# yuxng/PoseCNN

Hardware: NVIDIA H100
Metric: frames/sec on 640x480 RGB, 21 classes, batch 32 (VGG16 + Hough + ROI pose head) (higher is better)
Workload: dtype bf16 operands / fp32 accumulate (conv stack, 1x1 heads), fp16 operands / fp32 accumulate (fc6-fc8), fp32 / int32 elsewhere

## Files before the change

include/posecnn_b200.h:

```cpp
#ifndef POSECNN_B200_H_
#define POSECNN_B200_H_

#include <stddef.h>
#include <stdint.h>

#ifdef __cplusplus
extern "C" {
#endif

#define PCNN_OK 0
#define PCNN_E_INVALID (-1)
#define PCNN_E_WORKSPACE (-2)
#define PCNN_E_CUDA (-3)

#define PCNN_MAX_ROI 128
#define PCNN_HOUGH_MAX_ROWS (PCNN_MAX_ROI * 9)

const char* pcnn_last_error(void);
int pcnn_version(void);

int pcnn_hough_vote_workspace_bytes(int B, int H, int W, int C, int skip_pixels, float threshold_vote,
                                    size_t* bytes);
int pcnn_hough_vote_fwd(const int32_t* label, const float* vertex, const float* extents, const float* meta,
                        const float* gt, int B, int H, int W, int C, int num_gt, int num_meta, int is_train,
// ... 21 lines not shown
                           int height, int width, int channels, int pooled_height, int pooled_width,
                           float spatial_scale, float* top, int32_t* argmax, void* stream);
int pcnn_roi_pool_bwd(const float* top_diff, const int32_t* argmax, const float* rois, int batch, int num_rois,
                      int channel_rois, int height, int width, int channels, int pooled_height,
                      int pooled_width, float spatial_scale, int pool_channel, float* bottom_diff,
                      void* stream);

int pcnn_hard_label_fwd(const float* prob, const int32_t* gt, int B, int H, int W, int C, float threshold,
                        float* top, void* stream);
int pcnn_hard_label_bwd(int B, int H, int W, int C, float* grad_prob, float* grad_gt, void* stream);

int pcnn_backproject_fwd(const float* data, const float* label, const float* depth, const float* meta,
                         const float* label_3d, int B, int H, int W, int Cf, int C, int num_meta,
                         int grid_size, int kernel_size, float threshold, float* top_data, float* top_label,
                         float* top_flag, void* stream);
int pcnn_backproject_bwd(const float* top_diff, const float* depth, const float* meta, int B, int H, int W,
                         int Cf, int num_meta, int grid_size, float* bottom_diff, void* stream);

int pcnn_project_fwd(const float* data, const float* depth, const float* meta, int B, int H, int W, int Cf,
                     int num_meta, int grid_size, float* top, void* stream);
int pcnn_project_bwd(const float* top_diff, const float* depth, const float* meta, int B, int H, int W, int Cf,
                     int num_meta, int grid_size, int kernel_size, float threshold, float* bottom_diff,
                     void* stream);

int pcnn_average_distance_workspace_bytes(int N, size_t* bytes);
int pcnn_average_distance_fwd(const float* prediction, const float* target, const float* weight,
                              const float* point, const float* symmetry, int N, int C, int P, float margin,
                              float* loss, float* bottom_diff, void* workspace, size_t workspace_bytes,
                              void* stream);
int pcnn_average_distance_bwd(const float* top_diff, const float* bottom_diff, int N, int channels,
                              float* output, void* stream);

int pcnn_conv_bf16_tc(const void* in_bf16, const void* weights_bf16, const float* bias, void* out_bf16, int B,
                      int H, int W, int Cin, int Cout, int ksize, int relu, int block_n, void* stream);
int pcnn_conv_pool_bf16_tc(const void* in_bf16, const void* weights_bf16, const float* bias, void* out_pooled_bf16,
                           int B, int H, int W, int Cin, int Cout, int ksize, int relu, int block_n, void* stream);
int pcnn_conv3x3_small_cin(const float* in, const float* weights_hwio, const float* bias, void* out_bf16, int B,
                           int H, int W, int Cin, int Cout, int relu, void* stream);
int pcnn_im2col_c3(const void* in, int in_is_u8, const float* mean3_host, void* out_bf16, int B, int H, int W,
                   void* stream);
int pcnn_im2col_depth(const float* depth, const float* mean3_host, void* out_bf16, int B, int H, int W, void* stream);
int pcnn_conv1_fused_tc(const void* in, int in_is_u8, const float* mean3_host, const void* weights_bf16,
                        const float* bias, void* out_bf16, int B, int H, int W, int relu, void* stream);
int pcnn_conv1_depth_fused_tc(const float* depth, const float* mean3_host, const void* weights_bf16, const float* bias,
                              void* out_bf16, int B, int H, int W, int relu, void* stream);
int pcnn_maxpool2x2_bf16(const void* in_bf16, void* out_bf16, int B, int H, int W, int C, void* stream);

int pcnn_conv_wgrad_workspace_bytes(int B, int H, int W, int Cin, int Cout, int ksize, size_t* bytes);
int pcnn_conv_wgrad_bf16_tc(const void* x_bf16, const void* dz_bf16, int B, int H, int W, int Cin, int Cout, int ksize,
                            float scale, const float* w_f32, float decay, float* dW, void* workspace, size_t workspace_bytes,
                            void* stream);
int pcnn_fc_wgrad_f16_tc(const void* x_f16, const void* dy_f16, int rows, int Cin, int Cout, float scale, const float* w_f32,
                         float decay, float* dW, void* workspace, size_t workspace_bytes, void* stream);
int pcnn_bias_ws_bytes(int C, size_t* bytes);
int pcnn_relu_bwd_bf16(const void* g_bf16, const void* y_bf16, size_t npix, int C, int has_relu, void* dz_bf16, float scale,
                       const float* b, float decay, float* db, void* bias_ws, size_t bias_ws_bytes, void* stream);
int pcnn_maxpool_relu_bwd_bf16(const void* g_bf16, const void* y_bf16, int B, int H, int W, int C, void* dz_bf16, float scale,
                               const float* b, float decay, float* db, void* bias_ws, size_t bias_ws_bytes, void* stream);
int pcnn_add_to_bf16(const void* a_bf16, const void* b_bf16, const float* b_f32, size_t n, void* out_bf16, void* stream);

int pcnn_add_up2_bf16(const void* a4_bf16, const void* a5_bf16, int B, int h, int w, int C, void* out_bf16, void* stream);
int pcnn_up2_bwd_bf16(const void* dadd_bf16, const void* y5_bf16, int B, int h, int w, int C, void* d5_bf16, void* stream);
int pcnn_pack_lowres(const void* sc_bf16, int Cs, const void* vt_bf16, int Cv, int B, int h, int w, int C, float* lowres, void* stream);
int pcnn_up8_heads_bwd_ex(const float* prob, const float* score, const int32_t* gt, const float* cls_loss_out, float upstream_cls,
                          float threshold, const float* vertex_pred, const float* lowres, const float* bias_vertex, const float* centers,
                          const float* vertex_loss_out, float upstream_vertex, float w_inside, float sigma, int B, int h, int w, int C,
                          int Cs, int Cv, void* d_sc_bf16, void* d_vt_bf16, float* dbias, void* workspace, size_t workspace_bytes,
                          void* stream);
int pcnn_up8_heads_bwd_coord(const float* prob, const float* score, const int32_t* gt, const float* cls_loss_out, float upstream_cls,
// ... 123 lines not shown
```

posecnn_b200/conv.py:

```python
from __future__ import annotations

import torch

from ._lib import check, lib, ptr, stream


def hwio_to_tc(weights_hwio: torch.Tensor, dtype=torch.bfloat16) -> torch.Tensor:
    kh, kw, ci, co = weights_hwio.shape
    return weights_hwio.permute(3, 0, 1, 2).reshape(co, kh * kw * ci).to(dtype).contiguous()


def hwio_to_tc_dgrad(weights_hwio: torch.Tensor) -> torch.Tensor:
    kh, kw, ci, co = weights_hwio.shape
    flipped = torch.flip(weights_hwio, dims=(0, 1)).permute(0, 1, 3, 2).contiguous()
    return hwio_to_tc(flipped)


def conv_bf16(x: torch.Tensor, w_tc: torch.Tensor, bias: torch.Tensor, ksize: int, relu: bool, block_n: int = 0,
              out: torch.Tensor | None = None) -> torch.Tensor:
    assert x.is_cuda and x.dtype == torch.bfloat16 and x.is_contiguous() and x.dim() == 4
    assert w_tc.dtype == torch.bfloat16 and w_tc.is_contiguous() and bias.dtype == torch.float32
    B, H, W, Cin = x.shape
    Cout = w_tc.shape[0]
    assert w_tc.shape[1] == ksize * ksize * Cin
    if out is None:
        out = torch.empty((B, H, W, Cout), dtype=torch.bfloat16, device=x.device)
    check(lib().pcnn_conv_bf16_tc(ptr(x), ptr(w_tc), ptr(bias), ptr(out), B, H, W, Cin, Cout, int(ksize), int(bool(relu)),
                                  int(block_n), stream()))
    return out


def conv_pool_bf16(x: torch.Tensor, w_tc: torch.Tensor, bias: torch.Tensor, ksize: int, relu: bool, block_n: int = 0) -> torch.Tensor:
    assert x.is_cuda and x.dtype == torch.bfloat16 and x.is_contiguous() and x.dim() == 4
    B, H, W, Cin = x.shape
    Cout = w_tc.shape[0]
    out = torch.empty((B, H // 2, W // 2, Cout), dtype=torch.bfloat16, device=x.device)
    check(lib().pcnn_conv_pool_bf16_tc(ptr(x), ptr(w_tc), ptr(bias), ptr(out), B, H, W, Cin, Cout, int(ksize), int(bool(relu)),
                                       int(block_n), stream()))
    return out


def conv3x3_small_cin(x: torch.Tensor, w_hwio: torch.Tensor, bias: torch.Tensor, relu: bool = True) -> torch.Tensor:
    assert x.is_cuda and x.dtype == torch.float32 and x.is_contiguous()
    B, H, W, Cin = x.shape
    Cout = w_hwio.shape[3]
    out = torch.empty((B, H, W, Cout), dtype=torch.bfloat16, device=x.device)
    check(lib().pcnn_conv3x3_small_cin(ptr(x), ptr(w_hwio.contiguous()), ptr(bias), ptr(out), B, H, W, Cin, Cout,
                                       int(bool(relu)), stream()))
    return out


def maxpool2x2(x: torch.Tensor) -> torch.Tensor:
    assert x.is_cuda and x.dtype == torch.bfloat16 and x.is_contiguous()
    B, H, W, C = x.shape
    out = torch.empty((B, H // 2, W // 2, C), dtype=torch.bfloat16, device=x.device)
    check(lib().pcnn_maxpool2x2_bf16(ptr(x), ptr(out), B, H, W, C, stream()))
    return out


def im2col_c3(x: torch.Tensor, mean=None) -> torch.Tensor:
    import ctypes
    assert x.is_cuda and x.is_contiguous() and x.shape[3] == 3 and x.dtype in (torch.float32, torch.uint8)
# ... 45 lines not shown
```

posecnn_b200/csrc/conv_tc.cu:

```cuda
#include <cuda.h>
#include <cuda_bf16.h>

#include <type_traits>

#include "common.cuh"
#include "tc_common.cuh"

namespace pcnn {
namespace convtc {

constexpr int kTileH = 8, kTileW = 16;
static_assert(kTileH * kTileW == kTileM, "pixel tile = two wgmma M blocks");
constexpr int kABytes = kTileM * kKC * 2;
constexpr int kConsumers = 256;
constexpr int kProducerWarp = kConsumers / 32;
constexpr int kThreadsConv = kConsumers + 128;
constexpr int kConsumerRegs = 232, kProducerRegs = 40;
constexpr int kThreadsRow = kConsumers + 32;
constexpr int kStageBytes = 16 * 1024;

struct ConvParams {
    int B, H, W, Cin, Cout;
    int taps, ksize;
    int tiles_h, tiles_w, n_tiles_n, total_tiles;
    int tile_h, tile_w;
    int relu;
    int pool;
    int kc_outer;
    const float* bias;
};

__device__ __forceinline__ void consumer_sync() { asm volatile("bar.sync 1, 256;" ::: "memory"); }

__device__ __forceinline__ void release(uint64_t* bar, int lane)
{
    __syncwarp();
    if (lane == 0) mbar_arrive(bar);
}

__device__ __forceinline__ void stage_rows(uint8_t* ob, const float* a, const float* bias, int relu, int row, int q)
{
#pragma unroll
    for (int i = 0; i < 2; i++) {
        const int r = row + 8 * i;
#pragma unroll
        for (int jj = 0; jj < 8; jj++) {
            const int c = 8 * jj + 2 * q;
            float v0 = a[4 * jj + 2 * i] + __ldg(bias + c), v1 = a[4 * jj + 2 * i + 1] + __ldg(bias + c + 1);
            if (relu) { v0 = fmaxf(v0, 0.f); v1 = fmaxf(v1, 0.f); }
            *reinterpret_cast<uint32_t*>(ob + r * 128 + ((jj ^ (r & 7)) << 4) + 4 * q) = pack_bf16(v0, v1);
        }
    }
}

__device__ __forceinline__ void pool_staged(uint8_t* ob, int t)
{
    const int p = t >> 3, piece = t & 7;
    const int m = 32 * (p >> 3) + 2 * (p & 7);
    const int rows[4] = {m, m + 1, m + 16, m + 17};
    __nv_bfloat162 v[4];
    uint4 x = *reinterpret_cast<const uint4*>(ob + rows[0] * 128 + ((piece ^ (rows[0] & 7)) << 4));
    *reinterpret_cast<uint4*>(v) = x;
#pragma unroll
    for (int k = 1; k < 4; k++) {
        uint4 y = *reinterpret_cast<const uint4*>(ob + rows[k] * 128 + ((piece ^ (rows[k] & 7)) << 4));
        const __nv_bfloat162* yv = reinterpret_cast<const __nv_bfloat162*>(&y);
#pragma unroll
        for (int q = 0; q < 4; q++) v[q] = __hmax2(v[q], yv[q]);
    }
    consumer_sync();
    *reinterpret_cast<uint4*>(ob + p * 128 + ((piece ^ (p & 7)) << 4)) = *reinterpret_cast<const uint4*>(v);
}

template <int BN, int BM>
struct SmemPlan {
    static constexpr int kABytesT = BM * kKC * 2;
    static constexpr int kBBytes = BN * kKC * 2;
    static constexpr int kStage = kABytesT + kBBytes;
    static constexpr int kStages = BN == 256 || BM == 256 ? 4 : (BN == 128 ? 6 : 8);
    static constexpr int kOutBufs = 2;
    static constexpr int kBarOff = kStages * kStage + kOutBufs * kStageBytes;
    static constexpr int kTotal = kBarOff + 256 + 1024;
};

template <int BN, int BM>
__global__ void __launch_bounds__(kThreadsConv, 1)
k_conv_tc(const __grid_constant__ CUtensorMap map_in, const __grid_constant__ CUtensorMap map_w,
          const __grid_constant__ CUtensorMap map_out, const ConvParams p)
{
    static_assert(BM == 128 || (BM == 256 && BN <= 128), "k_conv_tc: BM = 256 needs BN <= 128 (accumulator registers)");
    using Plan = SmemPlan<BN, BM>;
    constexpr int kMB = BM / kTileM;
    extern __shared__ uint8_t smem_raw[];
    uint8_t* smem = reinterpret_cast<uint8_t*>((reinterpret_cast<uintptr_t>(smem_raw) + 1023) & ~(uintptr_t)1023);
    uint8_t* out_stage = smem + Plan::kStages * Plan::kStage;
    uint64_t* full = reinterpret_cast<uint64_t*>(smem + Plan::kBarOff);
    uint64_t* empty = full + Plan::kStages;

    const int warp = threadIdx.x >> 5, lane = threadIdx.x & 31;
    const int kchunks = p.Cin / kKC;
    const int ksteps = p.taps * kchunks;

    if (warp == kProducerWarp && lane == 0) {
        asm volatile("prefetch.tensormap [%0];" ::"l"(&map_in) : "memory");
        asm volatile("prefetch.tensormap [%0];" ::"l"(&map_w) : "memory");
        asm volatile("prefetch.tensormap [%0];" ::"l"(&map_out) : "memory");
        for (int s = 0; s < Plan::kStages; s++) { mbar_init(&full[s], 1); mbar_init(&empty[s], kConsumers / 32); }
        fence_barrier_init();
    }
    __syncthreads();

    if (warp >= kProducerWarp) {
        setmaxnreg_dec<kProducerRegs>();
        if (warp == kProducerWarp && elect_one()) {
            int stage = 0;
            uint32_t phase = 0;
            for (int tile = blockIdx.x; tile < p.total_tiles; tile += gridDim.x) {
                const int nt = tile % p.n_tiles_n;
                int rest = tile / p.n_tiles_n;
                const int tw = rest % p.tiles_w; rest /= p.tiles_w;
                const int th = rest % p.tiles_h;
                const int img = rest / p.tiles_h;
                const int h0 = th * p.tile_h, w0 = tw * p.tile_w, n0 = nt * BN;
                const int pad = p.ksize / 2;
#pragma unroll 1
                for (int ks = 0; ks < ksteps; ks++) {
                    const bool kc_outer = BM == 256 && p.kc_outer;
                    const int tap = kc_outer ? ks % p.taps : ks / kchunks;
                    const int c0 = (kc_outer ? ks / p.taps : ks % kchunks) * kKC;
                    const int dy = tap / p.ksize - pad, dx = tap % p.ksize - pad;
                    mbar_wait(&empty[stage], phase ^ 1);
                    uint8_t* sa = smem + stage * Plan::kStage;
                    mbar_arrive_expect_tx(&full[stage], Plan::kStage);
                    tma_load_4d(sa, &map_in, &full[stage], c0, w0 + dx, h0 + dy, img);
                    tma_load_2d(sa + Plan::kABytesT, &map_w, &full[stage], tap * p.Cin + c0, n0);
                    if (++stage == Plan::kStages) { stage = 0; phase ^= 1; }
                }
            }
        }
    } else {
        setmaxnreg_inc<kConsumerRegs>();
        const int wg = warp >> 2, wq = warp & 3;
        const int row = wg * 64 + wq * 16 + (lane >> 2);
        float acc[kMB][BN / 2];
        int stage = 0, obuf = 0;
        uint32_t phase = 0;
        for (int tile = blockIdx.x; tile < p.total_tiles; tile += gridDim.x) {
            const int nt = tile % p.n_tiles_n;
            int rest = tile / p.n_tiles_n;
            const int tw = rest % p.tiles_w; rest /= p.tiles_w;
            const int th = rest % p.tiles_h;
            const int img = rest / p.tiles_h;
            const int h0 = th * p.tile_h, w0 = tw * p.tile_w, n0 = nt * BN;
            int prev = -1;
            for (int ks = 0; ks < ksteps; ks++) {
                mbar_wait(&full[stage], phase);
                const uint32_t sa = smem_u32(smem + stage * Plan::kStage);
                const uint64_t db = make_desc(sa + Plan::kABytesT);
#pragma unroll
                for (int h = 0; h < kMB; h++) acc_fence<BN / 2>(acc[h]);
                wgmma_fence();
#pragma unroll
                for (int h = 0; h < kMB; h++) {
                    const uint64_t da = make_desc(sa + (h * 2 + wg) * 64 * 128);
#pragma unroll
                    for (int k = 0; k < kKC / 16; k++)
                        wgmma<BN, 0, 0, 0>(acc[h], da + (uint64_t)(k * 2), db + (uint64_t)(k * 2), (ks | k) != 0);
                }
                wgmma_commit();
#pragma unroll
                for (int h = 0; h < kMB; h++) acc_fence<BN / 2>(acc[h]);
                if (prev >= 0) {
                    wgmma_wait<1>();
                    release(&empty[prev], lane);
                }
                prev = stage;
                if (++stage == Plan::kStages) { stage = 0; phase ^= 1; }
            }
            wgmma_wait<0>();
#pragma unroll
            for (int h = 0; h < kMB; h++) acc_fence<BN / 2>(acc[h]);
            release(&empty[prev], lane);
#pragma unroll
            for (int h = 0; h < kMB; h++) {
                if (h > 0 && h0 + 8 * h >= p.H) break;
#pragma unroll
                for (int g = 0; g < BN / 64; g++) {
                    if (threadIdx.x == 0) tma_store_wait_read<1>();
                    consumer_sync();
                    uint8_t* ob = out_stage + obuf * kStageBytes;
                    stage_rows(ob, acc[h] + g * 32, p.bias + n0 + g * 64, p.relu, row, lane & 3);
                    if (p.pool) {
                        consumer_sync();
                        pool_staged(ob, threadIdx.x);
                    }
                    fence_proxy_async();
                    consumer_sync();
                    if (threadIdx.x == 0) {
                        if (!p.pool) tma_store_4d(&map_out, ob, n0 + g * 64, w0, h0 + 8 * h, img);
                        else tma_store_4d(&map_out, ob, n0 + g * 64, w0 >> 1, (h0 >> 1) + 4 * h, img);
                        tma_store_commit();
                    }
                    obuf ^= 1;
                }
            }
        }
        if (threadIdx.x == 0) tma_store_wait_all();
    }
}

constexpr int kRowPx = 128, kPatchW = 130, kPatchH = 4;
constexpr int kPatchBytes = kPatchW * kPatchH * 128;
constexpr int kRowAStages = 2;

template <int BN, bool RESB>
struct RowPlan {
    static constexpr int kBBytes = BN * 128;
    static constexpr int kBStages = RESB ? 9 : 6;
    static constexpr int kBOff = kRowAStages * kPatchBytes;
    static constexpr int kOutOff = kBOff + kBStages * kBBytes;
    static constexpr int kOutBytes = RESB ? kStageBytes : 2 * kStageBytes;
    static constexpr int kBarOff = kOutOff + kOutBytes;
    static constexpr int kTotal = kBarOff + 256 + 1024;
};

template <int BN, bool RESB>
__global__ void __launch_bounds__(kThreadsRow, 1)
k_conv_row2(const __grid_constant__ CUtensorMap map_in , const __grid_constant__ CUtensorMap map_w,
            const __grid_constant__ CUtensorMap map_out ,
            const ConvParams p)
{
    using Plan = RowPlan<BN, RESB>;
    static_assert(BN == 64, "row mode: 64-channel N tiles");
// ... 511 lines not shown
        const size_t n = r / Ho;
        const __nv_bfloat16* p0 = in + ((n * H + 2 * yo) * W + 2 * xo) * C + g * 8;
        uint4 a = __ldg(reinterpret_cast<const uint4*>(p0));
        uint4 b = __ldg(reinterpret_cast<const uint4*>(p0 + C));
        uint4 c = __ldg(reinterpret_cast<const uint4*>(p0 + (size_t)W * C));
        uint4 d = __ldg(reinterpret_cast<const uint4*>(p0 + (size_t)W * C + C));
        uint4 o;
        const __nv_bfloat162* pa = reinterpret_cast<const __nv_bfloat162*>(&a);
        const __nv_bfloat162* pb = reinterpret_cast<const __nv_bfloat162*>(&b);
        const __nv_bfloat162* pc = reinterpret_cast<const __nv_bfloat162*>(&c);
        const __nv_bfloat162* pd = reinterpret_cast<const __nv_bfloat162*>(&d);
        __nv_bfloat162* po = reinterpret_cast<__nv_bfloat162*>(&o);
#pragma unroll
        for (int k = 0; k < 4; k++) po[k] = __hmax2(__hmax2(pa[k], pb[k]), __hmax2(pc[k], pd[k]));
        *reinterpret_cast<uint4*>(out + ((n * Ho + yo) * Wo + xo) * C + g * 8) = o;
    }
}

static int make_map_nhwc(CUtensorMap* m, const void* ptr, int B, int H, int W, int C, int box_c, int box_w = kTileW, int box_h = kTileH)
{
    EncodeTiledFn enc = get_encode();
    if (!enc) { set_error("cuTensorMapEncodeTiled unavailable (driver too old?)"); return PCNN_E_CUDA; }
    cuuint64_t dims[4] = {(cuuint64_t)C, (cuuint64_t)W, (cuuint64_t)H, (cuuint64_t)B};
    cuuint64_t strides[3] = {(cuuint64_t)C * 2, (cuuint64_t)W * C * 2, (cuuint64_t)H * W * C * 2};
    cuuint32_t box[4] = {(cuuint32_t)box_c, (cuuint32_t)box_w, (cuuint32_t)box_h, 1};
    cuuint32_t es[4] = {1, 1, 1, 1};
    CUresult r = enc(m, CU_TENSOR_MAP_DATA_TYPE_BFLOAT16, 4, const_cast<void*>(ptr), dims, strides, box, es,
                     CU_TENSOR_MAP_INTERLEAVE_NONE, CU_TENSOR_MAP_SWIZZLE_128B, CU_TENSOR_MAP_L2_PROMOTION_L2_256B,
                     CU_TENSOR_MAP_FLOAT_OOB_FILL_NONE);
    if (r != CUDA_SUCCESS) { set_error("cuTensorMapEncodeTiled(NHWC %dx%dx%dx%d) failed: %d", B, H, W, C, (int)r); return PCNN_E_CUDA; }
    return PCNN_OK;
}

template <int BN, int BM = kTileM>
static int launch_conv(const CUtensorMap& mi, const CUtensorMap& mw, const CUtensorMap& mo, const ConvParams& p, int num_sms,
                       cudaStream_t st)
{
    using Plan = SmemPlan<BN, BM>;
    PCNN_SMEM_OPTIN((k_conv_tc<BN, BM>), Plan::kTotal, "conv_tc");
    int grid = p.total_tiles < num_sms ? p.total_tiles : num_sms;
    k_conv_tc<BN, BM><<<grid, kThreadsConv, Plan::kTotal, st>>>(mi, mw, mo, p);
    return check_launch("conv_tc");
}

template <int BN, bool RESB>
static int launch_conv_row2(const CUtensorMap& mi, const CUtensorMap& mw, const CUtensorMap& mo, const ConvParams& p, int num_sms,
                            cudaStream_t st)
{
    using Plan = RowPlan<BN, RESB>;
    PCNN_SMEM_OPTIN((k_conv_row2<BN, RESB>), Plan::kTotal, "conv_row2");
    int grid = p.total_tiles < num_sms ? p.total_tiles : num_sms;
    if (RESB) grid = grid / p.n_tiles_n * p.n_tiles_n;
    k_conv_row2<BN, RESB><<<grid, kThreadsRow, Plan::kTotal, st>>>(mi, mw, mo, p);
    return check_launch("conv_row2");
}

}
}

using namespace pcnn;
using namespace pcnn::convtc;

static int conv_bf16_tc_impl(const void* in, const void* weights, const float* bias, void* out, int B, int H, int W, int Cin,
                            int Cout, int ksize, int relu, int block_n, int pool, void* stream);

extern "C" int pcnn_conv_bf16_tc(const void* in, const void* weights, const float* bias, void* out, int B, int H, int W,
                                 int Cin, int Cout, int ksize, int relu, int block_n, void* stream)
{
    return conv_bf16_tc_impl(in, weights, bias, out, B, H, W, Cin, Cout, ksize, relu, block_n, 0, stream);
}

extern "C" int pcnn_conv_pool_bf16_tc(const void* in, const void* weights, const float* bias, void* out_pooled, int B, int H,
                                      int W, int Cin, int Cout, int ksize, int relu, int block_n, void* stream)
{
    PCNN_REQUIRE(H % 2 == 0 && W % 2 == 0, "conv_pool: needs even H, W (got %d x %d)", H, W);
    return conv_bf16_tc_impl(in, weights, bias, out_pooled, B, H, W, Cin, Cout, ksize, relu, block_n, 1, stream);
}

static int conv_bf16_tc_impl(const void* in, const void* weights, const float* bias, void* out, int B, int H, int W, int Cin,
                            int Cout, int ksize, int relu, int block_n, int pool, void* stream)
{
    PCNN_REQUIRE(in && weights && bias && out, "conv: NULL tensor pointer");
    PCNN_REQUIRE(ksize == 1 || ksize == 3, "conv: ksize must be 1 or 3 (got %d)", ksize);
    PCNN_REQUIRE(Cin % 64 == 0 && Cin >= 64, "conv: Cin must be a multiple of 64 (got %d)", Cin);
    PCNN_REQUIRE(Cout % 64 == 0 && Cout >= 64, "conv: Cout must be a multiple of 64 (got %d)", Cout);
    PCNN_REQUIRE(B >= 1 && H >= 1 && W >= 1, "conv: bad shape");
    int bn = block_n;
    if (bn == 0) bn = Cout % 256 == 0 && ksize * ksize * Cin >= 2304 ? 256 : (Cout % 128 == 0 ? 128 : 64);
    PCNN_REQUIRE((bn == 64 || bn == 128 || bn == 256) && Cout % bn == 0, "conv: block_n %d does not divide Cout %d", bn, Cout);
    int dev = 0, sms = kNumSMs;
    cudaGetDevice(&dev);
    cudaDeviceGetAttribute(&sms, cudaDevAttrMultiProcessorCount, dev);
    cudaStream_t st = (cudaStream_t)stream;
    CUtensorMap mi, mw, mo;
    int rc;
    const bool tile256 = block_n == 0 && ksize == 3 && Cin <= 128 && Cout == 128;
    if (block_n == 0 && ksize == 3 && Cin <= 128 && Cout == 64 && H % 2 == 0 && W >= kRowPx) {
        const bool resb = Cin == 64;
        bn = 64;
        rc = make_map_nhwc(&mi, in, B, H, W, Cin, kKC, kPatchW, kPatchH);
        if (rc) return rc;
        rc = make_map_weights(&mw, weights, 9 * Cin, Cout, bn);
        if (rc) return rc;
        rc = pool ? make_map_nhwc(&mo, out, B, H / 2, W / 2, Cout, 64, kRowPx / 2, 1) : make_map_nhwc(&mo, out, B, H, W, Cout, 64, kRowPx, 1);
        if (rc) return rc;
        ConvParams p;
        p.B = B; p.H = H; p.W = W; p.Cin = Cin; p.Cout = Cout; p.ksize = 3; p.taps = 9;
        p.tile_h = 2; p.tile_w = kRowPx;
        p.tiles_h = H / 2;
        p.tiles_w = (W + kRowPx - 1) / kRowPx;
        p.n_tiles_n = Cout / bn;
        p.total_tiles = B * p.tiles_h * p.tiles_w * p.n_tiles_n;
        p.relu = relu; p.pool = pool; p.bias = bias; p.kc_outer = 0;
        if (resb && p.total_tiles >= p.n_tiles_n) return launch_conv_row2<64, true>(mi, mw, mo, p, sms, st);
        return launch_conv_row2<64, false>(mi, mw, mo, p, sms, st);
    }
    int tile_h = kTileH, tile_w = kTileW;
    if (tile256) tile_h = 2 * kTileH;
    else if (!pool && ((H + 15) / 16) * ((W + 7) / 8) < ((H + 7) / 8) * ((W + 15) / 16)) { tile_h = 16; tile_w = 8; }
    rc = make_map_nhwc(&mi, in, B, H, W, Cin, kKC, tile_w, tile_h);
    if (rc) return rc;
    rc = make_map_weights(&mw, weights, ksize * ksize * Cin, Cout, bn);
    if (rc) return rc;
    rc = pool ? make_map_nhwc(&mo, out, B, H / 2, W / 2, Cout, 64, kTileW / 2, kTileH / 2)
              : make_map_nhwc(&mo, out, B, H, W, Cout, 64, tile_w, tile256 ? kTileH : tile_h);
    if (rc) return rc;
    ConvParams p;
    p.B = B; p.H = H; p.W = W; p.Cin = Cin; p.Cout = Cout;
    p.ksize = ksize; p.taps = ksize * ksize;
    p.tile_h = tile_h; p.tile_w = tile_w;
    p.tiles_h = (H + tile_h - 1) / tile_h;
    p.tiles_w = (W + tile_w - 1) / tile_w;
    p.n_tiles_n = Cout / bn;
    p.total_tiles = B * p.tiles_h * p.tiles_w * p.n_tiles_n;
    p.relu = relu;
    p.pool = pool;
    p.bias = bias;
    p.kc_outer = tile256 && H % 2 == 0 && W >= kRowPx;
    if (tile256) return launch_conv<128, 256>(mi, mw, mo, p, sms, st);
    if (bn == 256) return launch_conv<256>(mi, mw, mo, p, sms, st);
    if (bn == 128) return launch_conv<128>(mi, mw, mo, p, sms, st);
    return launch_conv<64>(mi, mw, mo, p, sms, st);
}

extern "C" int pcnn_conv3x3_small_cin(const float* in, const float* weights_hwio, const float* bias, void* out, int B, int H,
                                      int W, int Cin, int Cout, int relu, void* stream)
{
    PCNN_REQUIRE(in && weights_hwio && bias && out, "conv_small: NULL tensor pointer");
    PCNN_REQUIRE(Cin >= 1 && Cin <= 8 && Cout % 16 == 0 && Cout <= 128, "conv_small: needs Cin <= 8, Cout %% 16 == 0, Cout <= 128");
    size_t smem = sizeof(float) * (size_t)(9 * Cin + 1) * Cout;
    size_t total = (size_t)B * H * W * (Cout / 16);
    int blocks = (int)((total + 255) / 256 < (size_t)kNumSMs * 8 ? (total + 255) / 256 : (size_t)kNumSMs * 8);
    k_conv_small_cin<16><<<blocks, 256, smem, (cudaStream_t)stream>>>(in, weights_hwio, bias, (__nv_bfloat16*)out, B, H, W, Cin,
                                                                      Cout, relu);
    return check_launch("conv_small_cin");
}

extern "C" int pcnn_maxpool2x2_bf16(const void* in, void* out, int B, int H, int W, int C, void* stream)
{
    PCNN_REQUIRE(in && out, "maxpool: NULL tensor pointer");
    PCNN_REQUIRE(H % 2 == 0 && W % 2 == 0 && C % 8 == 0, "maxpool: needs even H, W and C %% 8 == 0 (got %d,%d,%d)", H, W, C);
    size_t total = (size_t)B * (H / 2) * (W / 2) * (C / 8);
    int blocks = (int)((total + 255) / 256 < (size_t)kNumSMs * 16 ? (total + 255) / 256 : (size_t)kNumSMs * 16);
    k_maxpool2x2_bf16<<<blocks, 256, 0, (cudaStream_t)stream>>>((const __nv_bfloat16*)in, (__nv_bfloat16*)out, B, H, W, C);
    return check_launch("maxpool2x2");
}

extern "C" int pcnn_im2col_c3(const void* in, int in_is_u8, const float* mean3_host, void* out_bf16, int B, int H, int W,
                              void* stream)
{
    PCNN_REQUIRE(in && out_bf16, "im2col: NULL tensor pointer");
    float m0 = 0.f, m1 = 0.f, m2 = 0.f;
    if (mean3_host) { m0 = mean3_host[0]; m1 = mean3_host[1]; m2 = mean3_host[2]; }
    PCNN_REQUIRE(H <= 65535 && B <= 65535, "im2col: image too tall for the launch grid");
    dim3 grid((W + 127) / 128, H, B);
// ... 21 lines not shown
                            const float* bias, void* out_bf16, int B, int H, int W, int relu, void* stream);

extern "C" int pcnn_conv1_fused_tc(const void* in, int in_is_u8, const float* mean3_host, const void* weights_bf16,
                                   const float* bias, void* out_bf16, int B, int H, int W, int relu, void* stream)
{
    return conv1_fused_impl(in, in_is_u8 ? 1 : 0, mean3_host, weights_bf16, bias, out_bf16, B, H, W, relu, stream);
}

extern "C" int pcnn_conv1_depth_fused_tc(const float* depth, const float* mean3_host, const void* weights_bf16,
                                         const float* bias, void* out_bf16, int B, int H, int W, int relu, void* stream)
{
    return conv1_fused_impl(depth, 2, mean3_host, weights_bf16, bias, out_bf16, B, H, W, relu, stream);
}

static int conv1_fused_impl(const void* in, int in_kind, const float* mean3_host, const void* weights_bf16,
                                   const float* bias, void* out_bf16, int B, int H, int W, int relu, void* stream)
{
    PCNN_REQUIRE(in && weights_bf16 && bias && out_bf16, "conv1: NULL tensor pointer");
    PCNN_REQUIRE(B >= 1 && H >= 1 && W >= 1, "conv1: bad shape");
    float m0 = 0.f, m1 = 0.f, m2 = 0.f;
    if (mean3_host) { m0 = mean3_host[0]; m1 = mean3_host[1]; m2 = mean3_host[2]; }
    CUtensorMap mw, mo;
    int rc = make_map_weights(&mw, weights_bf16, 64, 64, 64);
    if (rc) return rc;
    rc = make_map_nhwc(&mo, out_bf16, B, H, W, 64, 64);
    if (rc) return rc;
    ConvParams p;
    p.B = B; p.H = H; p.W = W; p.Cin = 3; p.Cout = 64; p.ksize = 3; p.taps = 9;
    p.tile_h = kTileH; p.tile_w = kTileW;
    p.tiles_h = (H + kTileH - 1) / kTileH;
    p.tiles_w = (W + kTileW - 1) / kTileW;
    p.n_tiles_n = 1;
    p.total_tiles = B * p.tiles_h * p.tiles_w;
    p.relu = relu; p.pool = 0; p.bias = bias; p.kc_outer = 0;
    int dev = 0, sms = kNumSMs;
    cudaGetDevice(&dev);
    cudaDeviceGetAttribute(&sms, cudaDevAttrMultiProcessorCount, dev);
    int grid = p.total_tiles < sms ? p.total_tiles : sms;
    cudaStream_t st = (cudaStream_t)stream;
    PCNN_SMEM_OPTIN(k_conv1_tc<unsigned char>, kC1Smem, "conv1_tc<u8>");
    PCNN_SMEM_OPTIN(k_conv1_tc<float>, kC1Smem, "conv1_tc<f32>");
    PCNN_SMEM_OPTIN(k_conv1_tc<DepthIn>, kC1Smem, "conv1_tc<depth>");
    if (in_kind == 1) k_conv1_tc<unsigned char><<<grid, kC1Threads, kC1Smem, st>>>((const unsigned char*)in, mw, mo, p, m0, m1, m2);
    else if (in_kind == 2) k_conv1_tc<DepthIn><<<grid, kC1Threads, kC1Smem, st>>>((const DepthIn*)in, mw, mo, p, m0, m1, m2);
    else k_conv1_tc<float><<<grid, kC1Threads, kC1Smem, st>>>((const float*)in, mw, mo, p, m0, m1, m2);
    return check_launch("conv1_fused_tc");
}
```

posecnn_b200/networks/trunk.py:

```python
from __future__ import annotations

import torch

from .. import conv

PIXEL_MEANS = (102.9801, 115.9465, 122.7717)

VGG_CFG = [("conv1_1", 3, 64), ("conv1_2", 64, 64), "pool1", ("conv2_1", 64, 128), ("conv2_2", 128, 128), "pool2",
           ("conv3_1", 128, 256), ("conv3_2", 256, 256), ("conv3_3", 256, 256), "pool3", ("conv4_1", 256, 512),
           ("conv4_2", 512, 512), ("conv4_3", 512, 512), "pool4", ("conv5_1", 512, 512), ("conv5_2", 512, 512),
           ("conv5_3", 512, 512)]


def trunk_shapes(sfx=""):
    shapes = {}
    for item in VGG_CFG:
        if isinstance(item, tuple):
            name, ci, co = item
            shapes[f"{name}{sfx}/weights"] = (3, 3, ci, co)
            shapes[f"{name}{sfx}/biases"] = (co,)
    return shapes


def conv_weights_to_tc(w: torch.Tensor) -> torch.Tensor:
    return conv.conv1_1_weights_to_tc(w) if w.shape[2] == 3 else conv.hwio_to_tc(w)


def run_trunk(P, T, data, sfx=""):
    if data.dim() == 3:
        x = conv.conv1_depth_fused(data, T[f"conv1_1{sfx}/weights"], P[f"conv1_1{sfx}/biases"], PIXEL_MEANS, True)
    else:
        mean = PIXEL_MEANS if data.dtype == torch.uint8 else None
        x = conv.conv1_fused(data, T[f"conv1_1{sfx}/weights"], P[f"conv1_1{sfx}/biases"], mean, True)
    feats = {}
    cfg = VGG_CFG[1:]
    i = 0
    while i < len(cfg):
        item = cfg[i]
        if isinstance(item, str):
            x = conv.maxpool2x2(x)
            i += 1
            continue
        name = item[0]
        fuse_pool = i + 1 < len(cfg) and isinstance(cfg[i + 1], str) and name not in ("conv4_3", "conv5_3")
        if fuse_pool:
            x = conv.conv_pool_bf16(x, T[f"{name}{sfx}/weights"], P[f"{name}{sfx}/biases"], 3, True)
            i += 2
            continue
        x = conv.conv_bf16(x, T[f"{name}{sfx}/weights"], P[f"{name}{sfx}/biases"], 3, True)
        if name in ("conv4_3", "conv5_3"):
            feats[name] = x
        i += 1
    return feats
```

Baseline: 2959.

## Fuse conv4_3 with pool4 via dual-output store and add paired 4x16 pixel tiles

Adds a dual-output conv path that writes both the full conv4_3 feature map and its 2x2 max-pooled version from the same staged epilogue, removing the separate maxpool kernel and its re-read of conv4_3. It also introduces a paired-block mode that stacks two 4x16 pixel tiles into one 128-row MMA tile to reduce padding waste on small feature maps such as conv5, plus a wave-quantization cost model for choosing BN 128 vs 256. The dual path gives up one pipeline stage of shared memory, and the new tile-selection heuristics can change which configuration the other layers use.

```diff
diff --git a/include/posecnn_b200.h b/include/posecnn_b200.h
--- a/include/posecnn_b200.h
+++ b/include/posecnn_b200.h
@@ -77,9 +77,12 @@
                               float* output, void* stream);
 
 int pcnn_conv_bf16_tc(const void* in_bf16, const void* weights_bf16, const float* bias, void* out_bf16, int B,
-                      int H, int W, int Cin, int Cout, int ksize, int relu, int block_n, void* stream);
+                      int H, int W, int Cin, int Cout, int ksize, int relu, int block_n, int pixel_tile, void* stream);
 int pcnn_conv_pool_bf16_tc(const void* in_bf16, const void* weights_bf16, const float* bias, void* out_pooled_bf16,
                            int B, int H, int W, int Cin, int Cout, int ksize, int relu, int block_n, void* stream);
+int pcnn_conv_dualpool_bf16_tc(const void* in_bf16, const void* weights_bf16, const float* bias, void* out_bf16,
+                               void* out_pooled_bf16, int B, int H, int W, int Cin, int Cout, int ksize, int relu, int block_n,
+                               int pixel_tile, void* stream);
 int pcnn_conv3x3_small_cin(const float* in, const float* weights_hwio, const float* bias, void* out_bf16, int B,
                            int H, int W, int Cin, int Cout, int relu, void* stream);
 int pcnn_im2col_c3(const void* in, int in_is_u8, const float* mean3_host, void* out_bf16, int B, int H, int W,
diff --git a/posecnn_b200/conv.py b/posecnn_b200/conv.py
--- a/posecnn_b200/conv.py
+++ b/posecnn_b200/conv.py
@@ -17,7 +17,7 @@
 
 
 def conv_bf16(x: torch.Tensor, w_tc: torch.Tensor, bias: torch.Tensor, ksize: int, relu: bool, block_n: int = 0,
-              out: torch.Tensor | None = None) -> torch.Tensor:
+              out: torch.Tensor | None = None, pixel_tile: int = 0) -> torch.Tensor:
     assert x.is_cuda and x.dtype == torch.bfloat16 and x.is_contiguous() and x.dim() == 4
     assert w_tc.dtype == torch.bfloat16 and w_tc.is_contiguous() and bias.dtype == torch.float32
     B, H, W, Cin = x.shape
@@ -26,8 +26,22 @@
     if out is None:
         out = torch.empty((B, H, W, Cout), dtype=torch.bfloat16, device=x.device)
     check(lib().pcnn_conv_bf16_tc(ptr(x), ptr(w_tc), ptr(bias), ptr(out), B, H, W, Cin, Cout, int(ksize), int(bool(relu)),
-                                  int(block_n), stream()))
+                                  int(block_n), int(pixel_tile), stream()))
     return out
+
+
+def conv_dualpool_bf16(x: torch.Tensor, w_tc: torch.Tensor, bias: torch.Tensor, ksize: int, relu: bool, block_n: int = 0,
+                       pixel_tile: int = 0) -> tuple[torch.Tensor, torch.Tensor]:
+    assert x.is_cuda and x.dtype == torch.bfloat16 and x.is_contiguous() and x.dim() == 4
+    assert w_tc.dtype == torch.bfloat16 and w_tc.is_contiguous() and bias.dtype == torch.float32
+    B, H, W, Cin = x.shape
+    Cout = w_tc.shape[0]
+    assert w_tc.shape[1] == ksize * ksize * Cin
+    out = torch.empty((B, H, W, Cout), dtype=torch.bfloat16, device=x.device)
+    pooled = torch.empty((B, H // 2, W // 2, Cout), dtype=torch.bfloat16, device=x.device)
+    check(lib().pcnn_conv_dualpool_bf16_tc(ptr(x), ptr(w_tc), ptr(bias), ptr(out), ptr(pooled), B, H, W, Cin, Cout, int(ksize),
+                                           int(bool(relu)), int(block_n), int(pixel_tile), stream()))
+    return out, pooled
 
 
 def conv_pool_bf16(x: torch.Tensor, w_tc: torch.Tensor, bias: torch.Tensor, ksize: int, relu: bool, block_n: int = 0) -> torch.Tensor:
diff --git a/posecnn_b200/csrc/conv_tc.cu b/posecnn_b200/csrc/conv_tc.cu
--- a/posecnn_b200/csrc/conv_tc.cu
+++ b/posecnn_b200/csrc/conv_tc.cu
@@ -24,6 +24,7 @@
     int taps, ksize;
     int tiles_h, tiles_w, n_tiles_n, total_tiles;
     int tile_h, tile_w;
+    int blocks;
     int relu;
     int pool;
     int kc_outer;
@@ -53,7 +54,7 @@
     }
 }
 
-__device__ __forceinline__ void pool_staged(uint8_t* ob, int t)
+__device__ __forceinline__ uint4 pool_piece(const uint8_t* ob, int t)
 {
     const int p = t >> 3, piece = t & 7;
     const int m = 32 * (p >> 3) + 2 * (p & 7);
@@ -68,32 +69,59 @@
 #pragma unroll
         for (int q = 0; q < 4; q++) v[q] = __hmax2(v[q], yv[q]);
     }
+    return *reinterpret_cast<const uint4*>(v);
+}
+
+__device__ __forceinline__ void store_pooled_piece(uint8_t* dst, int t, uint4 v)
+{
+    const int p = t >> 3, piece = t & 7;
+    *reinterpret_cast<uint4*>(dst + p * 128 + ((piece ^ (p & 7)) << 4)) = v;
+}
+
+__device__ __forceinline__ void pool_staged(uint8_t* ob, int t)
+{
+    const uint4 v = pool_piece(ob, t);
     consumer_sync();
-    *reinterpret_cast<uint4*>(ob + p * 128 + ((piece ^ (p & 7)) << 4)) = *reinterpret_cast<const uint4*>(v);
-}
-
-template <int BN, int BM>
+    store_pooled_piece(ob, t, v);
+}
+
+__device__ __forceinline__ void tile_origin(const ConvParams& p, int idx, int& img, int& h0, int& w0)
+{
+    const int tw = idx % p.tiles_w;
+    const int rest = idx / p.tiles_w;
+    h0 = (rest % p.tiles_h) * p.tile_h;
+    w0 = tw * p.tile_w;
+    img = rest / p.tiles_h;
+}
+
+template <int BN, int BM, bool DUAL = false>
 struct SmemPlan {
     static constexpr int kABytesT = BM * kKC * 2;
     static constexpr int kBBytes = BN * kKC * 2;
     static constexpr int kStage = kABytesT + kBBytes;
-    static constexpr int kStages = BN == 256 || BM == 256 ? 4 : (BN == 128 ? 6 : 8);
+    static constexpr int kStages = (BN == 256 || BM == 256 ? 4 : (BN == 128 ? 6 : 8)) - (DUAL ? 1 : 0);
     static constexpr int kOutBufs = 2;
-    static constexpr int kBarOff = kStages * kStage + kOutBufs * kStageBytes;
+    static constexpr int kPoolBytes = kStageBytes / 4;
+    static constexpr int kPoolOff = kStages * kStage + kOutBufs * kStageBytes;
+    static constexpr int kBarOff = kPoolOff + (DUAL ? kOutBufs * kPoolBytes : 0);
     static constexpr int kTotal = kBarOff + 256 + 1024;
 };
 
-template <int BN, int BM>
+template <int BN, int BM, bool DUAL = false>
 __global__ void __launch_bounds__(kThreadsConv, 1)
 k_conv_tc(const __grid_constant__ CUtensorMap map_in, const __grid_constant__ CUtensorMap map_w,
-          const __grid_constant__ CUtensorMap map_out, const ConvParams p)
-{
-    static_assert(BM == 128 || (BM == 256 && BN <= 128), "k_conv_tc: BM = 256 needs BN <= 128 (accumulator registers)");
-    using Plan = SmemPlan<BN, BM>;
+          const __grid_constant__ CUtensorMap map_out,
+          const __grid_constant__ CUtensorMap map_pool,
+          const ConvParams p)
+{
+    static_assert(BM == 128 || (BM == 256 && BN <= 128 && !DUAL), "k_conv_tc: BM = 256 needs BN <= 128 (accumulator registers)");
+    using Plan = SmemPlan<BN, BM, DUAL>;
     constexpr int kMB = BM / kTileM;
     extern __shared__ uint8_t smem_raw[];
     uint8_t* smem = reinterpret_cast<uint8_t*>((reinterpret_cast<uintptr_t>(smem_raw) + 1023) & ~(uintptr_t)1023);
     uint8_t* out_stage = smem + Plan::kStages * Plan::kStage;
+    uint8_t* pool_stage = smem + Plan::kPoolOff;
+    const bool blocks = BM == 128 && p.blocks > 0;
     uint64_t* full = reinterpret_cast<uint64_t*>(smem + Plan::kBarOff);
     uint64_t* empty = full + Plan::kStages;
 
@@ -105,6 +133,7 @@
         asm volatile("prefetch.tensormap [%0];" ::"l"(&map_in) : "memory");
         asm volatile("prefetch.tensormap [%0];" ::"l"(&map_w) : "memory");
         asm volatile("prefetch.tensormap [%0];" ::"l"(&map_out) : "memory");
+        if (DUAL) asm volatile("prefetch.tensormap [%0];" ::"l"(&map_pool) : "memory");
         for (int s = 0; s < Plan::kStages; s++) { mbar_init(&full[s], 1); mbar_init(&empty[s], kConsumers / 32); }
         fence_barrier_init();
     }
@@ -116,12 +145,14 @@
             int stage = 0;
             uint32_t phase = 0;
             for (int tile = blockIdx.x; tile < p.total_tiles; tile += gridDim.x) {
-                const int nt = tile % p.n_tiles_n;
-                int rest = tile / p.n_tiles_n;
-                const int tw = rest % p.tiles_w; rest /= p.tiles_w;
-                const int th = rest % p.tiles_h;
-                const int img = rest / p.tiles_h;
-                const int h0 = th * p.tile_h, w0 = tw * p.tile_w, n0 = nt * BN;
+                const int nt = tile % p.n_tiles_n, pt = tile / p.n_tiles_n, n0 = nt * BN;
+                int img, h0, w0, img1 = 0, h1 = 0, w1 = 0;
+                if (blocks) {
+                    tile_origin(p, 2 * pt, img, h0, w0);
+                    tile_origin(p, min(2 * pt + 1, p.blocks - 1), img1, h1, w1);
+                } else {
+                    tile_origin(p, pt, img, h0, w0);
+                }
                 const int pad = p.ksize / 2;
 #pragma unroll 1
                 for (int ks = 0; ks < ksteps; ks++) {
@@ -133,6 +164,7 @@
                     uint8_t* sa = smem + stage * Plan::kStage;
                     mbar_arrive_expect_tx(&full[stage], Plan::kStage);
                     tma_load_4d(sa, &map_in, &full[stage], c0, w0 + dx, h0 + dy, img);
+                    if (blocks) tma_load_4d(sa + kABytes / 2, &map_in, &full[stage], c0, w1 + dx, h1 + dy, img1);
                     tma_load_2d(sa + Plan::kABytesT, &map_w, &full[stage], tap * p.Cin + c0, n0);
                     if (++stage == Plan::kStages) { stage = 0; phase ^= 1; }
                 }
@@ -146,12 +178,9 @@
         int stage = 0, obuf = 0;
         uint32_t phase = 0;
         for (int tile = blockIdx.x; tile < p.total_tiles; tile += gridDim.x) {
-            const int nt = tile % p.n_tiles_n;
-            int rest = tile / p.n_tiles_n;
-            const int tw = rest % p.tiles_w; rest /= p.tiles_w;
-            const int th = rest % p.tiles_h;
-            const int img = rest / p.tiles_h;
-            const int h0 = th * p.tile_h, w0 = tw * p.tile_w, n0 = nt * BN;
+            const int nt = tile % p.n_tiles_n, pt = tile / p.n_tiles_n, n0 = nt * BN;
+            int img, h0, w0;
+            tile_origin(p, blocks ? 2 * pt : pt, img, h0, w0);
             int prev = -1;
             for (int ks = 0; ks < ksteps; ks++) {
                 mbar_wait(&full[stage], phase);
@@ -189,16 +218,31 @@
                     if (threadIdx.x == 0) tma_store_wait_read<1>();
                     consumer_sync();
                     uint8_t* ob = out_stage + obuf * kStageBytes;
+                    uint8_t* pb = pool_stage + obuf * Plan::kPoolBytes;
                     stage_rows(ob, acc[h] + g * 32, p.bias + n0 + g * 64, p.relu, row, lane & 3);
-                    if (p.pool) {
+                    if (DUAL) {
+                        consumer_sync();
+                        store_pooled_piece(pb, threadIdx.x, pool_piece(ob, threadIdx.x));
+                    } else if (p.pool) {
                         consumer_sync();
                         pool_staged(ob, threadIdx.x);
                     }
                     fence_proxy_async();
                     consumer_sync();
                     if (threadIdx.x == 0) {
-                        if (!p.pool) tma_store_4d(&map_out, ob, n0 + g * 64, w0, h0 + 8 * h, img);
-                        else tma_store_4d(&map_out, ob, n0 + g * 64, w0 >> 1, (h0 >> 1) + 4 * h, img);
+                        const int c = n0 + g * 64;
+                        if (blocks) {
+                            for (int b = 0; b < 2 && 2 * pt + b < p.blocks; b++) {
+                                int bi, bh, bw;
+                                tile_origin(p, 2 * pt + b, bi, bh, bw);
+                                tma_store_4d(&map_out, ob + b * (kStageBytes / 2), c, bw, bh, bi);
+                                if (DUAL) tma_store_4d(&map_pool, pb + b * (Plan::kPoolBytes / 2), c, bw >> 1, bh >> 1, bi);
+                            }
+                        } else {
+                            if (p.pool == 1) tma_store_4d(&map_out, ob, c, w0 >> 1, (h0 >> 1) + 4 * h, img);
+                            else tma_store_4d(&map_out, ob, c, w0, h0 + 8 * h, img);
+                            if (DUAL) tma_store_4d(&map_pool, pb, c, w0 >> 1, (h0 >> 1) + 4 * h, img);
+                        }
                         tma_store_commit();
                     }
                     obuf ^= 1;
@@ -776,15 +820,29 @@
     return PCNN_OK;
 }
 
-template <int BN, int BM = kTileM>
-static int launch_conv(const CUtensorMap& mi, const CUtensorMap& mw, const CUtensorMap& mo, const ConvParams& p, int num_sms,
-                       cudaStream_t st)
-{
-    using Plan = SmemPlan<BN, BM>;
-    PCNN_SMEM_OPTIN((k_conv_tc<BN, BM>), Plan::kTotal, "conv_tc");
+template <int BN, int BM = kTileM, bool DUAL = false>
+static int launch_conv(const CUtensorMap& mi, const CUtensorMap& mw, const CUtensorMap& mo, const CUtensorMap& mp,
+                       const ConvParams& p, int num_sms, cudaStream_t st)
+{
+    using Plan = SmemPlan<BN, BM, DUAL>;
+    static_assert(Plan::kTotal <= 232448, "k_conv_tc: shared memory above the sm_90 opt-in");
+    PCNN_SMEM_OPTIN((k_conv_tc<BN, BM, DUAL>), Plan::kTotal, "conv_tc");
     int grid = p.total_tiles < num_sms ? p.total_tiles : num_sms;
-    k_conv_tc<BN, BM><<<grid, kThreadsConv, Plan::kTotal, st>>>(mi, mw, mo, p);
+    k_conv_tc<BN, BM, DUAL><<<grid, kThreadsConv, Plan::kTotal, st>>>(mi, mw, mo, mp, p);
     return check_launch("conv_tc");
+}
+
+constexpr double kCostBN128 = 1.017;
+constexpr int kMinWavesForBNRule = 8;
+
+static int conv_default_bn(long pixel_tiles, int Cout, int K, int sms)
+{
+    if (!(Cout % 256 == 0 && K >= 2304)) return Cout % 128 == 0 ? 128 : 64;
+    const long items256 = pixel_tiles * (Cout / 256), items128 = 2 * items256;
+    if (items256 < (long)kMinWavesForBNRule * sms) return 256;
+    const double cost256 = (double)((items256 + sms - 1) / sms) * 256;
+    const double cost128 = (double)((items128 + sms - 1) / sms) * 128 * kCostBN128;
+    return cost128 < cost256 ? 128 : 256;
 }
 
 template <int BN, bool RESB>
@@ -805,41 +863,53 @@
 using namespace pcnn;
 using namespace pcnn::convtc;
 
-static int conv_bf16_tc_impl(const void* in, const void* weights, const float* bias, void* out, int B, int H, int W, int Cin,
-                            int Cout, int ksize, int relu, int block_n, int pool, void* stream);
+static int conv_bf16_tc_impl(const void* in, const void* weights, const float* bias, void* out, void* out_pooled, int B, int H,
+                             int W, int Cin, int Cout, int ksize, int relu, int block_n, int pixel_tile, int pool, void* stream);
 
 extern "C" int pcnn_conv_bf16_tc(const void* in, const void* weights, const float* bias, void* out, int B, int H, int W,
-                                 int Cin, int Cout, int ksize, int relu, int block_n, void* stream)
-{
-    return conv_bf16_tc_impl(in, weights, bias, out, B, H, W, Cin, Cout, ksize, relu, block_n, 0, stream);
+                                 int Cin, int Cout, int ksize, int relu, int block_n, int pixel_tile, void* stream)
+{
+    return conv_bf16_tc_impl(in, weights, bias, out, nullptr, B, H, W, Cin, Cout, ksize, relu, block_n, pixel_tile, 0, stream);
 }
 
 extern "C" int pcnn_conv_pool_bf16_tc(const void* in, const void* weights, const float* bias, void* out_pooled, int B, int H,
                                       int W, int Cin, int Cout, int ksize, int relu, int block_n, void* stream)
 {
     PCNN_REQUIRE(H % 2 == 0 && W % 2 == 0, "conv_pool: needs even H, W (got %d x %d)", H, W);
-    return conv_bf16_tc_impl(in, weights, bias, out_pooled, B, H, W, Cin, Cout, ksize, relu, block_n, 1, stream);
-}
-
-static int conv_bf16_tc_impl(const void* in, const void* weights, const float* bias, void* out, int B, int H, int W, int Cin,
-                            int Cout, int ksize, int relu, int block_n, int pool, void* stream)
+    return conv_bf16_tc_impl(in, weights, bias, out_pooled, nullptr, B, H, W, Cin, Cout, ksize, relu, block_n, 0, 1, stream);
+}
+
+extern "C" int pcnn_conv_dualpool_bf16_tc(const void* in, const void* weights, const float* bias, void* out, void* out_pooled,
+                                          int B, int H, int W, int Cin, int Cout, int ksize, int relu, int block_n, int pixel_tile,
+                                          void* stream)
+{
+    PCNN_REQUIRE(H % 2 == 0 && W % 2 == 0, "conv_dualpool: needs even H, W (got %d x %d)", H, W);
+    PCNN_REQUIRE(out_pooled, "conv_dualpool: NULL tensor pointer");
+    return conv_bf16_tc_impl(in, weights, bias, out, out_pooled, B, H, W, Cin, Cout, ksize, relu, block_n, pixel_tile, 2, stream);
+}
+
+static int conv_bf16_tc_impl(const void* in, const void* weights, const float* bias, void* out, void* out_pooled, int B, int H,
+                             int W, int Cin, int Cout, int ksize, int relu, int block_n, int pixel_tile, int pool, void* stream)
 {
     PCNN_REQUIRE(in && weights && bias && out, "conv: NULL tensor pointer");
     PCNN_REQUIRE(ksize == 1 || ksize == 3, "conv: ksize must be 1 or 3 (got %d)", ksize);
     PCNN_REQUIRE(Cin % 64 == 0 && Cin >= 64, "conv: Cin must be a multiple of 64 (got %d)", Cin);
     PCNN_REQUIRE(Cout % 64 == 0 && Cout >= 64, "conv: Cout must be a multiple of 64 (got %d)", Cout);
     PCNN_REQUIRE(B >= 1 && H >= 1 && W >= 1, "conv: bad shape");
+    PCNN_REQUIRE(block_n == 0 || ((block_n == 64 || block_n == 128 || block_n == 256) && Cout % block_n == 0),
+                 "conv: block_n %d does not divide Cout %d", block_n, Cout);
+    PCNN_REQUIRE(pixel_tile == 0 || pixel_tile == 64 || pixel_tile == 128, "conv: pixel_tile must be 0, 64 or 128 (got %d)", pixel_tile);
+    PCNN_REQUIRE(pool != 1 || pixel_tile != 64, "conv_pool: the pool-only store runs on the 8 x 16 tile");
     int bn = block_n;
-    if (bn == 0) bn = Cout % 256 == 0 && ksize * ksize * Cin >= 2304 ? 256 : (Cout % 128 == 0 ? 128 : 64);
-    PCNN_REQUIRE((bn == 64 || bn == 128 || bn == 256) && Cout % bn == 0, "conv: block_n %d does not divide Cout %d", bn, Cout);
     int dev = 0, sms = kNumSMs;
     cudaGetDevice(&dev);
     cudaDeviceGetAttribute(&sms, cudaDevAttrMultiProcessorCount, dev);
     cudaStream_t st = (cudaStream_t)stream;
     CUtensorMap mi, mw, mo;
     int rc;
-    const bool tile256 = block_n == 0 && ksize == 3 && Cin <= 128 && Cout == 128;
-    if (block_n == 0 && ksize == 3 && Cin <= 128 && Cout == 64 && H % 2 == 0 && W >= kRowPx) {
+    const bool open = block_n == 0 && pixel_tile == 0 && pool != 2;
+    const bool tile256 = open && ksize == 3 && Cin <= 128 && Cout == 128;
+    if (open && ksize == 3 && Cin <= 128 && Cout == 64 && H % 2 == 0 && W >= kRowPx) {
         const bool resb = Cin == 64;
         bn = 64;
         rc = make_map_nhwc(&mi, in, B, H, W, Cin, kKC, kPatchW, kPatchH);
@@ -855,36 +925,58 @@
         p.tiles_w = (W + kRowPx - 1) / kRowPx;
         p.n_tiles_n = Cout / bn;
         p.total_tiles = B * p.tiles_h * p.tiles_w * p.n_tiles_n;
-        p.relu = relu; p.pool = pool; p.bias = bias; p.kc_outer = 0;
+        p.relu = relu; p.pool = pool; p.bias = bias; p.kc_outer = 0; p.blocks = 0;
         if (resb && p.total_tiles >= p.n_tiles_n) return launch_conv_row2<64, true>(mi, mw, mo, p, sms, st);
         return launch_conv_row2<64, false>(mi, mw, mo, p, sms, st);
     }
     int tile_h = kTileH, tile_w = kTileW;
-    if (tile256) tile_h = 2 * kTileH;
-    else if (!pool && ((H + 15) / 16) * ((W + 7) / 8) < ((H + 7) / 8) * ((W + 15) / 16)) { tile_h = 16; tile_w = 8; }
-    rc = make_map_nhwc(&mi, in, B, H, W, Cin, kKC, tile_w, tile_h);
-    if (rc) return rc;
-    rc = make_map_weights(&mw, weights, ksize * ksize * Cin, Cout, bn);
-    if (rc) return rc;
-    rc = pool ? make_map_nhwc(&mo, out, B, H / 2, W / 2, Cout, 64, kTileW / 2, kTileH / 2)
-              : make_map_nhwc(&mo, out, B, H, W, Cout, 64, tile_w, tile256 ? kTileH : tile_h);
-    if (rc) return rc;
+    bool blk = false;
+    if (tile256) {
+        tile_h = 2 * kTileH;
+    } else {
+        const long px816 = (long)((H + 7) / 8) * ((W + 15) / 16) * 128, px168 = (long)((H + 15) / 16) * ((W + 7) / 8) * 128;
+        const long px416 = (long)((H + 3) / 4) * ((W + 15) / 16) * 64;
+        blk = pool != 1 && (pixel_tile == 64 || (pixel_tile == 0 && px416 < px816 && (pool || px416 < px168)));
+        if (blk) tile_h = 4;
+        else if (!pool && px168 < px816) { tile_h = 16; tile_w = 8; }
+    }
     ConvParams p;
     p.B = B; p.H = H; p.W = W; p.Cin = Cin; p.Cout = Cout;
     p.ksize = ksize; p.taps = ksize * ksize;
     p.tile_h = tile_h; p.tile_w = tile_w;
     p.tiles_h = (H + tile_h - 1) / tile_h;
     p.tiles_w = (W + tile_w - 1) / tile_w;
+    p.blocks = blk ? B * p.tiles_h * p.tiles_w : 0;
+    const long pixel_tiles = blk ? (p.blocks + 1) / 2 : (long)B * p.tiles_h * p.tiles_w;
+    if (tile256) bn = 128;
+    else if (bn == 0) bn = conv_default_bn(pixel_tiles, Cout, ksize * ksize * Cin, sms);
     p.n_tiles_n = Cout / bn;
-    p.total_tiles = B * p.tiles_h * p.tiles_w * p.n_tiles_n;
+    p.total_tiles = (int)(pixel_tiles * p.n_tiles_n);
+    rc = make_map_nhwc(&mi, in, B, H, W, Cin, kKC, tile_w, tile_h);
+    if (rc) return rc;
+    rc = make_map_weights(&mw, weights, ksize * ksize * Cin, Cout, bn);
+    if (rc) return rc;
+    rc = pool == 1 ? make_map_nhwc(&mo, out, B, H / 2, W / 2, Cout, 64, kTileW / 2, kTileH / 2)
+                   : make_map_nhwc(&mo, out, B, H, W, Cout, 64, tile_w, tile256 ? kTileH : tile_h);
+    if (rc) return rc;
+    CUtensorMap mp = mo;
+    if (pool == 2) {
+        rc = make_map_nhwc(&mp, out_pooled, B, H / 2, W / 2, Cout, 64, tile_w / 2, tile_h / 2);
+        if (rc) return rc;
+    }
     p.relu = relu;
     p.pool = pool;
     p.bias = bias;
     p.kc_outer = tile256 && H % 2 == 0 && W >= kRowPx;
-    if (tile256) return launch_conv<128, 256>(mi, mw, mo, p, sms, st);
-    if (bn == 256) return launch_conv<256>(mi, mw, mo, p, sms, st);
-    if (bn == 128) return launch_conv<128>(mi, mw, mo, p, sms, st);
-    return launch_conv<64>(mi, mw, mo, p, sms, st);
+    if (tile256) return launch_conv<128, 256>(mi, mw, mo, mp, p, sms, st);
+    if (pool == 2) {
+        if (bn == 256) return launch_conv<256, kTileM, true>(mi, mw, mo, mp, p, sms, st);
+        if (bn == 128) return launch_conv<128, kTileM, true>(mi, mw, mo, mp, p, sms, st);
+        return launch_conv<64, kTileM, true>(mi, mw, mo, mp, p, sms, st);
+    }
+    if (bn == 256) return launch_conv<256>(mi, mw, mo, mp, p, sms, st);
+    if (bn == 128) return launch_conv<128>(mi, mw, mo, mp, p, sms, st);
+    return launch_conv<64>(mi, mw, mo, mp, p, sms, st);
 }
 
 extern "C" int pcnn_conv3x3_small_cin(const float* in, const float* weights_hwio, const float* bias, void* out, int B, int H,
@@ -972,7 +1064,7 @@
     p.tiles_w = (W + kTileW - 1) / kTileW;
     p.n_tiles_n = 1;
     p.total_tiles = B * p.tiles_h * p.tiles_w;
-    p.relu = relu; p.pool = 0; p.bias = bias; p.kc_outer = 0;
+    p.relu = relu; p.pool = 0; p.bias = bias; p.kc_outer = 0; p.blocks = 0;
     int dev = 0, sms = kNumSMs;
     cudaGetDevice(&dev);
     cudaDeviceGetAttribute(&sms, cudaDevAttrMultiProcessorCount, dev);
diff --git a/posecnn_b200/networks/trunk.py b/posecnn_b200/networks/trunk.py
--- a/posecnn_b200/networks/trunk.py
+++ b/posecnn_b200/networks/trunk.py
@@ -42,7 +42,11 @@
             i += 1
             continue
         name = item[0]
-        fuse_pool = i + 1 < len(cfg) and isinstance(cfg[i + 1], str) and name not in ("conv4_3", "conv5_3")
+        fuse_pool = i + 1 < len(cfg) and isinstance(cfg[i + 1], str)
+        if fuse_pool and name == "conv4_3":
+            feats[name], x = conv.conv_dualpool_bf16(x, T[f"{name}{sfx}/weights"], P[f"{name}{sfx}/biases"], 3, True)
+            i += 2
+            continue
         if fuse_pool:
             x = conv.conv_pool_bf16(x, T[f"{name}{sfx}/weights"], P[f"{name}{sfx}/biases"], 3, True)
             i += 2
```

Result: no change. 2944, median of 6 (-0.5%).
